# raw-lab/mercat2

Hardware: AMD Instinct MI355X
Metric: bases/sec at k=31, 10Mx150bp (higher is better)
Workload: dtype u64

## Files before the change

### mercat2_amd/csrc/mk_skmer.hip

```cpp
#include "mk_skmer_dev.h"
#include <cstdlib>
#include <cstdio>
#include <vector>
#include <type_traits>

#define SK_NKMAX 8
#ifndef SK_HIST_THREADS
#define SK_HIST_THREADS 256
#endif
#ifndef SK_HIST_GRID
#define SK_HIST_GRID 512
#endif
#ifndef SK_SCAT_GRID
#define SK_SCAT_GRID 4096
#endif
#define SK_MAX_P1_LOG2 13
#define SK_MAX_P1 (1 << SK_MAX_P1_LOG2)
#ifndef SK_BUCKET_SYMS
#define SK_BUCKET_SYMS 8192
#endif
#define SK_NOFIT 0xFF000000u

template <int W, class F>
__device__ __forceinline__ void sk_for_each_record(u64 w0, u64 w1, u64 badw, int k, int nkmax, bool canon, F&& emit) {
  const SkRuns r = sk_analyse<W>(w0, w1, sk_valid32(badw, k), canon);
  sk_walk(r, w0, w1, nkmax, canon, emit);
}

__device__ __forceinline__ ulonglong2 sk_make_record(u64 w0, u64 w1, int jstart, int nk, int k) {
  const int s = 2 * jstart;
  u64 hi = (w0 << s) | ((w1 >> 1) >> (63 - s));
  u64 lo = w1 << s;
  const int t = 2 * (nk + k - 1);
  const u64 mh = t >= 64 ? ~0ull : (~0ull << ((64 - t) & 63));
  const u64 ml = t <= 64 ? 0ull : (~0ull << ((128 - t) & 63));
  hi &= mh;
  lo = (lo & ml) | (u64)nk;
  return make_ulonglong2(hi, lo);
}

template <int W, bool CANON>
__global__ __launch_bounds__(SK_HIST_THREADS) void mk_sk_hist_k(const u64* __restrict__ codes, const u64* __restrict__ bad,
                                                                const MkChunkInfo* __restrict__ info, u64* __restrict__ hist,
                                                                u64* __restrict__ khist, int p1_log2, int k, int nkmax,
                                                                size_t nthreads_total, int canon, int sample_log2) {
  extern __shared__ unsigned sk_hist_lds[];
  (void)canon;
  sk_hist_body(sk_hist_lds, sk_hist_lds + (1u << p1_log2), info, hist, p1_log2, nthreads_total, sample_log2,
               [&](size_t t, size_t p0, auto&& tally) {
                 sk_for_each_record<W>(codes[t], codes[t + 1], bad_window(bad, p0), k, nkmax, CANON, tally);
               });
}

#ifndef SK_TU_CANON
__device__ __forceinline__ u64 sk_cap(u64 h, int sample_log2, u64 weight, float sigmas) {
  if (sample_log2 == 0) return h;
  const u64 est = h << sample_log2;
  const float dev = sigmas * __builtin_sqrtf((float)((u64)weight << sample_log2) * (float)est);
  return est + (u64)dev + 1 + (sigmas > 0 ? 16 * weight : 0);
}
__device__ __forceinline__ u64 sk_seg_cap(u64 h, int sample_log2, u64 weight, float sigmas, int nseg) {
  const float est = (float)(h << sample_log2);
  const float var = (float)weight * est * (1.0f / (float)nseg + (float)(1u << sample_log2) / (float)(nseg * nseg));
  return (u64)(est / (float)nseg) + (u64)(sigmas * __builtin_sqrtf(var)) + 1 + (sigmas > 0 ? 4 * weight : 0);
}
__global__ __launch_bounds__(1024) void mk_sk_scan_k(const u64* __restrict__ hist, const u64* __restrict__ khist,
                                                     u64* __restrict__ start, SkCursor* __restrict__ cursor, u64* __restrict__ kstart,
                                                     MkChunkInfo* __restrict__ info, int p1_log2, int sample_log2, int nkmax,
                                                     u64 div, u64 part_cap, u64 surv_cap, float sigmas, int nseg) {
  constexpr int PER = SK_MAX_P1 / 1024;
  __shared__ u64 wsum[16], wksum[16];
  const unsigned p1 = 1u << p1_log2;
  const unsigned per = (p1 + 1023) / 1024;
  const unsigned lo = threadIdx.x * per;
  const int lane = threadIdx.x & 63, wv = threadIdx.x >> 6;
  u64 cap[PER], kcap[PER];
  u64 acc = 0, kacc = 0;
#pragma unroll
  for (int q = 0; q < PER; ++q) {
    const unsigned i = lo + q;
    const bool on = (unsigned)q < per && i < p1;
    const u64 hk = on ? hist[i] : 0ull;
    cap[q] = !on ? 0 : (nseg > 1 ? sk_seg_cap(hk & 0xFFFFFFFFull, sample_log2, SK_R / SK_NKMAX, sigmas, 8)
                                 : sk_cap(hk & 0xFFFFFFFFull, sample_log2, SK_R / SK_NKMAX, sigmas));
    kcap[q] = on ? (sk_cap(hk >> 32, sample_log2, SK_R, sigmas) + div - 1) / div : 0;
    acc += cap[q];
    kacc += kcap[q];
  }
  u64 inc = acc, kinc = kacc;
#pragma unroll
  for (int d = 1; d < 64; d <<= 1) {
    const u64 a = __shfl_up(inc, d), b = __shfl_up(kinc, d);
    if (lane >= d) { inc += a; kinc += b; }
  }
  if (lane == 63) { wsum[wv] = inc; wksum[wv] = kinc; }
  __syncthreads();
  u64 run = inc - acc, krun = kinc - kacc;
  for (int w = 0; w < wv; ++w) { run += wsum[w]; krun += wksum[w]; }
  __shared__ u64 s_total;
  if (threadIdx.x == 1023) {
    const u64 total = run + acc, ktotal = krun + kacc;
    s_total = total;
    const u64 all = nseg > 1 ? 16 * total : total;
    start[(size_t)nseg * p1] = all;
    kstart[p1] = ktotal;
    if (all > part_cap) atomicOr(&info->part_overflow, 1ull);
    if (ktotal > surv_cap) atomicOr(&info->part_overflow, 2ull);
  }
  __shared__ unsigned s_run[SK_MAX_P1];
#pragma unroll
  for (int q = 0; q < PER; ++q) {
    const unsigned i = lo + q;
    if ((unsigned)q < per && i < p1) {
      s_run[i] = (unsigned)run;
      kstart[i] = krun;
      run += cap[q];
      krun += kcap[q];
    }
  }
  __syncthreads();
  const u64 total = s_total;
  for (int x = 0; x < nseg; ++x)
    for (unsigned i = threadIdx.x; i < p1; i += 1024) {
      const u64 at = x < 8 ? (u64)x * total + s_run[i] : 8 * total + 8 * (u64)s_run[i];
      start[(size_t)x * p1 + i] = at;
      cursor[(size_t)x * p1 + i] = (SkCursor)at;
    }
}

#endif

#ifdef MK_STAMP
static __device__ u64 skq_dbg[1024 * 8];
#endif
#define SKQ_CAP 512
#if defined(SK_ABL_COARSE) && !defined(SK_PLAIN_CURSORS)
#error "SK_ABL_COARSE needs -DSK_PLAIN_CURSORS (the ablation's region ends differ from the ones sk_reserve8k checks)"
#endif
#ifndef SKQ_THREADS
#define SKQ_THREADS 512
#endif
#define SKQ_WAVES (SKQ_THREADS / 64)
#define SKQ_WALKED 0xFFFFFFFFu
template <int W, bool CANON, int SKQ_SUBT, int SKQ_QCAP>
__global__ __launch_bounds__(SKQ_THREADS) __attribute__((amdgpu_waves_per_eu(4, 4))) void mk_sk_scatterq_k(const u64* __restrict__ codes, const u64* __restrict__ bad,
                                                         MkChunkInfo* __restrict__ info, const u64* __restrict__ start,
                                                         SkCursor* __restrict__ cursor, ulonglong2* __restrict__ part,
                                                         int p1_log2, int k, int nkmax, size_t ntiles, unsigned qcap, int nseg) {
  SkCursor* const shared_cursor = cursor + ((size_t)8 << p1_log2);
  const u64* const shared_start = start + ((size_t)8 << p1_log2);
  if (nseg > 1) {
    unsigned xcc;
    asm volatile("s_getreg_b32 %0, hwreg(HW_REG_XCC_ID)" : "=s"(xcc));
    const size_t seg = xcc & 7u;
    cursor += seg << p1_log2;
    start += seg << p1_log2;
  }
  __shared__ unsigned lh[SK_MAX_P1];
  __shared__ u64 pk_x[SKQ_SUBT][SKQ_WAVES][65];
  __shared__ unsigned queue[SKQ_SUBT][SKQ_WAVES][SKQ_QCAP];
  __shared__ unsigned s_abort;
  if (threadIdx.x == 0) s_abort = info->part_overflow != 0;
  __syncthreads();
  if (s_abort) return;
  unsigned spilled = 0;
  constexpr int NB = SK_MAX_P1 / SKQ_THREADS;
  const unsigned p1 = 1u << p1_log2;
  const size_t seq_len = info->seq_len;
  const int lane = threadIdx.x & 63;
#define wv sk_wave_id()
  auto sk_wave_id = [&]() { int w = (int)threadIdx.x; asm volatile("" : "+v"(w)); return w >> 6; };
  for (unsigned i = threadIdx.x; i < p1; i += blockDim.x) lh[i] = 0;
  __syncthreads();
  u64 tA = 0, tB = 0, tC = 0, tD = 0, tE = 0, tF = 0, t0 = 0, ntile = 0;
  (void)tA; (void)tB; (void)tC; (void)tD; (void)tE; (void)tF; (void)t0; (void)ntile;
  STAMP(t0);
  for (size_t tile = blockIdx.x; tile < ntiles; tile += gridDim.x) {
    ntile += 1;
    unsigned qn[SKQ_SUBT];
#pragma unroll
    for (int st = 0; st < SKQ_SUBT; ++st) {
      const size_t t = (tile * SKQ_SUBT + st) * SKQ_THREADS + threadIdx.x;
      const size_t p0 = t * SK_R;
      SkRuns runs;
      runs.valid = 0;
      runs.starts = 0;
      runs.pos[0] = runs.pos[1] = runs.pos[2] = runs.pos[3] = 0;
      u64 ww0 = 0, ww1 = 0;
      if (p0 < seq_len) {
        ww0 = codes[t];
        ww1 = codes[t + 1];
        runs = sk_analyse<W>(ww0, ww1, sk_valid32(bad_window(bad, p0), k), CANON);
      } else if (p0 < seq_len + SK_R) {
        ww0 = codes[t];
      }
      pk_x[st][wv][lane] = ww0;
      if (lane == 63) pk_x[st][wv][64] = ww1;
      const unsigned s2 = sk_cut_starts(runs.starts, runs.valid, nkmax);
      const unsigned cnt = __popc(s2);
      const unsigned inc = mk_wave_scan_incl(cnt);
      const unsigned total = mk_wave_last(inc);
      unsigned* const myq = queue[st][wv];
      if (total <= qcap) {
        unsigned todo = s2, at = inc - cnt;
        while (todo) {
          const int j = __ffs(todo) - 1;
          todo &= todo - 1;
          const unsigned stop = (s2 | ~runs.valid) & ~((2u << j) - 1);
          const int nk = (stop ? (__ffs(stop) - 1) : SK_R) - j;
          const u64 pw = j < 10 ? runs.pos[0] : (j < 20 ? runs.pos[1] : (j < 30 ? runs.pos[2] : runs.pos[3]));
          const unsigned best = (unsigned)(pw >> (6 * (j % 10))) & 63u;
          myq[at++] = (unsigned)lane | ((unsigned)j << 6) | ((unsigned)nk << 11) | (best << 16);
        }
        __builtin_amdgcn_fence(__ATOMIC_RELEASE, "wavefront");
        __builtin_amdgcn_wave_barrier();
        __builtin_amdgcn_fence(__ATOMIC_ACQUIRE, "wavefront");
        for (unsigned base = 0; base < total; base += 64) {
          const unsigned i = base + lane;
          if (i < total) {
            const unsigned it = myq[i];
            const u64* const wp = &pk_x[st][wv][it & 63u];
            const unsigned mm = sk_canon_mmer(sk_mmer(wp[0], wp[1], (int)(it >> 16)), CANON);
#ifdef SK_ABL_COARSE
            const unsigned b = sk_bucket(mm, p1_log2) & ~63u;
#else
            const unsigned b = sk_bucket(mm, p1_log2);
#endif
            atomicAdd(&lh[b], 1u);
            myq[i] = (it & 0xFFFFu) | (b << 16);
          }
        }
        qn[st] = total;
      } else {
        if (p0 < seq_len)
          sk_walk(runs, ww0, ww1, nkmax, CANON, [&](int, int, unsigned mm) {
            atomicAdd(&lh[sk_bucket(mm, p1_log2)], 1u);
          });
        qn[st] = SKQ_WALKED;
      }
    }
    STAMP_ADD(tA, t0);
    __syncthreads();
    STAMP_ADD(tB, t0);
    unsigned roff = 0;
    asm volatile("" : "+s"(roff));
    SkCursor* const rcursor = cursor + roff;
    const u64* const rstart = start + roff;
    SkCursor* const rshared_cursor = shared_cursor + roff;
    const u64* const rshared_start = shared_start + roff;
#ifndef SK_PLAIN_CURSORS
    if (p1 == SK_MAX_P1) {
      static_assert(NB % 8 == 0, "sk_reserve8");
#pragma unroll
      for (int h = 0; h < NB; h += 8) {
        unsigned v[8], at[8];
#pragma unroll
        for (int i = 0; i < 8; ++i) v[i] = lh[threadIdx.x + (h + i) * SKQ_THREADS];
        unsigned nofit = sk_reserve8<SKQ_THREADS>(v, rcursor + h * SKQ_THREADS, rstart + h * SKQ_THREADS, SK_NOFIT, at);
        if (nseg > 1 && __any(nofit)) {
          unsigned v2[8], at2[8];
#pragma unroll
          for (int i = 0; i < 8; ++i) {
            v2[i] = at[i] >= SK_NOFIT ? v[i] : 0u;
            const unsigned pad = at[i] >= SK_NOFIT ? at[i] & 0xFFFFFFu : 0u;
            if (pad) {
              const u64 end = rstart[threadIdx.x + (h + i) * SKQ_THREADS + 1];
              for (unsigned q = 0; q < pad; ++q) part[end - pad + q] = make_ulonglong2(0, 0);
            }
          }
          nofit = sk_reserve8<SKQ_THREADS>(v2, rshared_cursor + h * SKQ_THREADS, rshared_start + h * SKQ_THREADS, SK_NOFIT, at2);
#pragma unroll
          for (int i = 0; i < 8; ++i) at[i] = v2[i] ? at2[i] : at[i];
        }
        spilled |= nofit;
#pragma unroll
        for (int i = 0; i < 8; ++i) lh[threadIdx.x + (h + i) * SKQ_THREADS] = at[i];
      }
    } else
#endif
    {
      for (unsigned b = threadIdx.x; b < p1; b += SKQ_THREADS) {
        const unsigned v = lh[b];
        u64 r = v ? (u64)atomicAdd(&rcursor[b], v) : 0ull;
#ifdef SK_ABL_COARSE
        const bool fits = v == 0 || r + v <= rstart[b + 64 < p1 ? b + 64 : p1];
#else
        bool fits = v == 0 || r + v <= rstart[b + 1];
        if (!fits && nseg > 1) {
          for (u64 q = r; q < rstart[b + 1]; ++q) part[q] = make_ulonglong2(0, 0);
          r = (u64)atomicAdd(&rshared_cursor[b], v);
          fits = r + v <= rshared_start[b + 1];
        }
#endif
        spilled |= fits ? 0u : 1u;
        lh[b] = fits ? (unsigned)r : SK_NOFIT;
      }
    }
    STAMP_ADD(tC, t0);
    __syncthreads();
    STAMP_ADD(tD, t0);
#pragma unroll
    for (int st = 0; st < SKQ_SUBT; ++st) {
      if (qn[st] != SKQ_WALKED) {
        const unsigned total = qn[st];
        const unsigned* const myq = queue[st][wv];
        for (unsigned base = 0; base < total; base += 64) {
          const unsigned i = base + lane;
          if (i < total) {
            const unsigned it = myq[i];
            const unsigned at = atomicAdd(&lh[it >> 16], 1u);
            const u64* const wp = &pk_x[st][wv][it & 63u];
            ulonglong2 rec = sk_make_record(wp[0], wp[1], (int)((it >> 6) & 31u), (int)((it >> 11) & 31u), k);
            asm volatile("" : "+v"(rec.x), "+v"(rec.y));
            if (at < SK_NOFIT) part[(size_t)at] = rec;
          }
        }
      } else {
        const size_t t = (tile * SKQ_SUBT + st) * SKQ_THREADS + threadIdx.x;
        const size_t p0 = t * SK_R;
        if (p0 < seq_len) {
          const ulonglong2 w = make_ulonglong2(pk_x[st][wv][lane], pk_x[st][wv][lane + 1]);
          const SkRuns runs = sk_analyse<W>(w.x, w.y, sk_valid32(bad_window(bad, p0), k), CANON);
          sk_walk(runs, w.x, w.y, nkmax, CANON, [&](int jstart, int nk, unsigned mm) {
            const unsigned at = atomicAdd(&lh[sk_bucket(mm, p1_log2)], 1u);
            if (at < SK_NOFIT) part[(size_t)at] = sk_make_record(w.x, w.y, jstart, nk, k);
          });
        }
      }
    }
    STAMP_ADD(tE, t0);
    __syncthreads();
    for (unsigned i = threadIdx.x; i < p1; i += blockDim.x) lh[i] = 0;
    __syncthreads();
    STAMP_ADD(tF, t0);
  }
#ifdef MK_STAMP
  if (threadIdx.x == 0 && blockIdx.x < 1024) { u64* d = skq_dbg + (size_t)blockIdx.x * 8; d[0] = tA; d[1] = tB; d[2] = tC; d[3] = tD; d[4] = tE; d[5] = tF; d[6] = ntile; }
#endif
  if (spilled) atomicOr(&info->part_overflow, 4ull);
}
#undef wv


#ifndef SK_TU_CANON
void mk_launch_sk_scan(mk_ctx* c, const u64* hist, const u64* khist, u64* start, SkCursor* cursor, u64* kstart, int p1_log2,
                       int sample_log2, int nkmax, u64 surv_div, u64 part_cap, u64 surv_cap, float sigmas, int nseg) {
  hipLaunchKernelGGL(mk_sk_scan_k, dim3(1), dim3(1024), 0, c->stream, hist, khist, start, cursor, kstart,
                     (MkChunkInfo*)c->info.p, p1_log2, sample_log2, nkmax, surv_div, part_cap, surv_cap, sigmas, nseg);
}

#endif

template <int W, bool CANON>
static void launch_wc(mk_ctx* c, size_t seq_len, int p1_log2, int nkmax, int sample_log2, u64 surv_div, u64 part_cap, u64 surv_cap,
                     u64* hist, u64* start, SkCursor* cursor, u64* khist, u64* kstart, bool reuse, int nseg) {
  MkChunkInfo* info = (MkChunkInfo*)c->info.p;
  const size_t threads = div_up(seq_len, SK_R);
  const size_t tiles = div_up(div_up(threads, (size_t)1 << sample_log2), SK_HIST_THREADS);
  const size_t hist_grid = sample_log2 ? SK_HIST_GRID / 2 : SK_HIST_GRID;
  if (!reuse) {
    const float sigmas = (float)mk_env_double("MK_SAMPLE_SIGMAS", 6.0);
    hipLaunchKernelGGL((mk_sk_hist_k<W, CANON>), dim3((unsigned)(tiles < hist_grid ? tiles : hist_grid)), dim3(SK_HIST_THREADS),
                       2 * sizeof(unsigned) << p1_log2, c->stream,
                       (const u64*)c->codes.p, (const u64*)c->bad.p, info, hist, khist, p1_log2, c->k, nkmax, threads, c->canonical,
                       sample_log2);
    mk_launch_sk_scan(c, (const u64*)hist, (const u64*)khist, start, cursor, kstart, p1_log2, sample_log2, nkmax, surv_div, part_cap,
                      surv_cap, sigmas, nseg);
  }
  const SkQueueShape shape = sk_queue_shape(c);
  const bool three = shape.three;
  const unsigned qcap = shape.qcap;
  const size_t qtiles = div_up(threads, (size_t)SKQ_THREADS * (three ? 3 : 2));
  const dim3 qgrid((unsigned)(qtiles < SK_SCAT_GRID ? qtiles : SK_SCAT_GRID));
  if (three)
    hipLaunchKernelGGL((mk_sk_scatterq_k<W, CANON, 3, 376>), qgrid, dim3(SKQ_THREADS), 0, c->stream, (const u64*)c->codes.p,
                       (const u64*)c->bad.p, info, (const u64*)start, cursor, (ulonglong2*)c->part.p, p1_log2, c->k, nkmax, qtiles, qcap, nseg);
  else
    hipLaunchKernelGGL((mk_sk_scatterq_k<W, CANON, 2, 512>), qgrid, dim3(SKQ_THREADS), 0, c->stream, (const u64*)c->codes.p,
                       (const u64*)c->bad.p, info, (const u64*)start, cursor, (ulonglong2*)c->part.p, p1_log2, c->k, nkmax, qtiles, qcap, nseg);
#ifdef MK_STAMP
  {
    (void)hipStreamSynchronize(c->stream);
    const unsigned g = qgrid.x;
    std::vector<u64> h(8 * 1024);
    (void)hipMemcpyFromSymbol(h.data(), HIP_SYMBOL(skq_dbg), h.size() * 8);
    double a[7] = {0, 0, 0, 0, 0, 0, 0};
    for (unsigned w = 0; w < g && w < 1024; ++w) for (int q = 0; q < 7; ++q) a[q] += (double)h[w * 8 + q] / g;
    fprintf(stderr, "[stamp scatterq] per WG (wave 0): analyse+list+pass1=%.0f barrier1=%.0f cursors=%.0f barrier2=%.0f pass2=%.0f barrier3+clear=%.0f tiles=%.2f grid=%u\n",
            a[0], a[1], a[2], a[3], a[4], a[5], a[6], g);
  }
#endif
}


template <bool CANON>
static bool sk_partition(int W, mk_ctx* c, size_t seq_len, int p1_log2, int nkmax, int sample_log2, u64 surv_div, u64 part_cap, u64 surv_cap,
                         u64* hist, u64* start, SkCursor* cursor, u64* khist, u64* kstart, bool reuse, int nseg) {
  switch (W) {
#define SK_CASE(W_)                                                                                                      \
  case W_: launch_wc<W_, CANON>(c, seq_len, p1_log2, nkmax, sample_log2, surv_div, part_cap, surv_cap, hist, start, cursor, khist, kstart, reuse, nseg); return true;
    SK_CASE(2) SK_CASE(3) SK_CASE(4) SK_CASE(5) SK_CASE(6) SK_CASE(7)
    SK_CASE(8) SK_CASE(9) SK_CASE(10) SK_CASE(11) SK_CASE(12) SK_CASE(13) SK_CASE(14) SK_CASE(15) SK_CASE(16)
    SK_CASE(17) SK_CASE(18) SK_CASE(19) SK_CASE(20) SK_CASE(21) SK_CASE(22)
#undef SK_CASE
    default: return false;
  }
}

#ifdef SK_TU_CANON
bool mk_sk_partition_canon(int W, mk_ctx* c, size_t seq_len, int p1_log2, int nkmax, int sample_log2, u64 surv_div, u64 part_cap,
                           u64 surv_cap, u64* hist, u64* start, SkCursor* cursor, u64* khist, u64* kstart, bool reuse, int nseg) {
  return sk_partition<true>(W, c, seq_len, p1_log2, nkmax, sample_log2, surv_div, part_cap, surv_cap, hist, start, cursor, khist, kstart, reuse, nseg);
}
#else
bool mk_sk_partition_canon(int W, mk_ctx* c, size_t seq_len, int p1_log2, int nkmax, int sample_log2, u64 surv_div, u64 part_cap,
                           u64 surv_cap, u64* hist, u64* start, SkCursor* cursor, u64* khist, u64* kstart, bool reuse, int nseg);

bool mk_part_inherit(mk_ctx* c, size_t seq_len, int p1_log2, uint64_t min_count, bool sampled, bool exact) {
  if (c->part_cooldown > 0 && !exact) c->part_cooldown -= 1;
  const bool reuse = !exact && sampled && c->part_reuse_ok && !c->part_dirty && c->part_cooldown == 0 &&
                     p1_log2 == c->part_prev_p1 && (unsigned long long)min_count == c->part_prev_minc &&
                     seq_len <= c->part_prev_len + c->part_prev_len / 100 && seq_len >= c->part_prev_len - c->part_prev_len / 50 &&
                     !mk_env_set("MK_NO_REUSE");
  if (reuse) c->st.part_reused += 1;
  c->part_dirty = true;
  if (exact) { c->part_reuse_ok = false; c->part_cooldown = 4; }
  else if (sampled && !reuse) {
    c->part_reuse_ok = true;
    c->part_prev_len = seq_len;
    c->part_prev_p1 = p1_log2;
    c->part_prev_minc = (unsigned long long)min_count;
  } else if (!reuse) c->part_reuse_ok = false;
  return reuse;
}

int sk_p1_log2(size_t seq_len, int max_log2, size_t bucket_syms) {
  int p1_log2 = 8;
  while (p1_log2 < max_log2 && (seq_len >> p1_log2) > bucket_syms) ++p1_log2;
  return p1_log2;
}
int sk_sample_log2(size_t seq_len, bool exact) {
  return !exact && seq_len >= (size_t)mk_env_int("MK_SAMPLE_MIN", (long long)8 << 20) ? 3 : 0;
}
u64 sk_surv_div(uint64_t min_count) { return min_count > 1 ? (u64)min_count : 1; }
size_t sk_surv_cap(size_t seq_len, size_t p1, u64 surv_div, int sample_log2) {
  if (!sample_log2) return seq_len / surv_div + p1 + 64;
  const double L = 1.25 * (double)seq_len, S = (double)(1u << sample_log2), w = (double)SK_R;
  return (size_t)((L + 6.0 * sqrt((double)p1 * S * w * L) + 16.0 * w * (double)p1) / (double)surv_div) + 2 * p1 + 64;
}
SkQueueShape sk_queue_shape(const mk_ctx* c) {
  const long long force_subt = mk_env_int("MK_SKQ_SUBT", 0);
  SkQueueShape q;
  q.three = force_subt == 3 || (force_subt != 2 && c->items_hint > 0 && c->items_hint * 64.0 + 48.0 < 376.0);
  q.qcap = q.three ? 376u : 512u;
  { const long long v = mk_env_int("MK_SKQ_CAP", -1); if (v >= 0 && (unsigned long long)v < q.qcap) q.qcap = (unsigned)v; }
  return q;
}

int mk_launch_count_superkmer(mk_ctx* c, size_t seq_len, uint64_t min_count, bool exact) {
  if (seq_len == 0) return MK_OK;
  const int k = c->k;
  const int p1_log2 = sk_p1_log2(seq_len, SK_MAX_P1_LOG2, SK_BUCKET_SYMS);
  c->p1_log2 = p1_log2;
  const size_t p1 = (size_t)1 << p1_log2;
  int nkmax = 62 - k;
  if (nkmax > SK_NKMAX) nkmax = SK_NKMAX;
  { const long long v = mk_env_int("MK_NKMAX", 0); if (v >= 1 && v <= 31 && v <= 62 - k) nkmax = (int)v; }
  const int sample_log2 = sk_sample_log2(seq_len, exact);
  c->part_sampled = sample_log2 != 0;
  const int nseg = (sample_log2 != 0 && seq_len <= ((size_t)1 << 30) && mk_env_int("MK_XSEG", 1) != 0) ? 9 : 1;
  if (nseg != c->part_nseg) c->part_reuse_ok = false;
  c->part_nseg = nseg;
  const bool reuse = mk_part_inherit(c, seq_len, p1_log2, min_count, sample_log2 != 0, exact);
  int rc;
  if ((rc = mk_buf_reserve(c, c->part_meta, sk_meta_words(p1, SKC_SEG_MAX) * sizeof(u64))) != MK_OK) return rc;
  const size_t part_cap = nseg > 1 ? 2 * seq_len + 64 : seq_len + 64;
  if ((rc = mk_buf_reserve(c, c->part, part_cap * sizeof(ulonglong2))) != MK_OK) return rc;
  const u64 surv_div = sk_surv_div(min_count);
  const size_t surv_cap = sk_surv_cap(seq_len, p1, surv_div, sample_log2);
  if ((rc = mk_buf_reserve(c, c->surv_keys, surv_cap * sizeof(u64))) != MK_OK) return rc;
  if ((rc = mk_buf_reserve(c, c->surv_cnts, surv_cap * sizeof(u64))) != MK_OK) return rc;
  const SkMeta m = sk_meta(c->part_meta.p, p1, nseg);
  if (!reuse) MK_HIP(hipMemsetAsync(m.hist, 0, sk_meta_cleared_words(p1) * sizeof(u64), c->stream));
  mk_prof_begin(c, MK_K_PART);
  if (c->canonical) {
    if (!mk_sk_partition_canon(k - SK_M + 1, c, seq_len, p1_log2, nkmax, sample_log2, surv_div, (u64)part_cap, (u64)surv_cap, m.hist, m.start, m.cursor, m.khist, m.kstart, reuse, nseg)) {
      c->err = "mk_launch_count_superkmer: k out of range";
      return MK_ERR_ARG;
    }
  } else if (!sk_partition<false>(k - SK_M + 1, c, seq_len, p1_log2, nkmax, sample_log2, surv_div, (u64)part_cap, (u64)surv_cap, m.hist, m.start, m.cursor, m.khist, m.kstart, reuse, nseg)) {
    c->err = "mk_launch_count_superkmer: k out of range";
    return MK_ERR_ARG;
  }
  mk_prof_end(c);
  if ((rc = mk_launch_sk_count(c, (const u64*)m.start, m.cursor, (const u64*)m.kstart, m.nsurv, min_count, p1, nseg)) != MK_OK) return rc;
  MK_HIP(hipGetLastError());
  c->surv_regions = 1;
  return MK_OK;
}
#endif
```

### mercat2_amd/csrc/mk_skmer_dev.h

```cpp
#pragma once
#include "mk_common.h"
#include "mk_device.h"

#define SK_M 11
#define SK_MASK ((1u << (2 * SK_M)) - 1)
#define SK_R 32

__device__ __forceinline__ unsigned sk_order_raw(unsigned mm) {
  return __umul24(mm, 0x9277B5u) + 0x2C5A3Du;
}
__device__ __forceinline__ unsigned sk_order_hash(unsigned mm) { return sk_order_raw(mm) & SK_MASK; }
__device__ __forceinline__ unsigned sk_canon_mmer(unsigned mm, bool canon) {
  if (!canon) return mm;
  const unsigned rc = (unsigned)mk_revcomp2((u64)mm, SK_M);
  return rc < mm ? rc : mm;
}
__device__ __forceinline__ unsigned sk_bucket(unsigned mm, int p1_log2) { return (mm * 0xC2B2AE3Du) >> (32 - p1_log2); }

__device__ __forceinline__ unsigned sk_mmer(u64 w0, u64 w1, int q) {
  const u64 a = q < 32 ? w0 : w1, b = q < 32 ? w1 : 0ull;
  const int s = 2 * (q & 31);
  const u64 x = (a << s) | ((b >> 1) >> (63 - s));
  return (unsigned)(x >> (64 - 2 * SK_M));
}

typedef unsigned SkCursor;

#ifndef SK_PLAIN_CURSORS
template <int THREADS>
__device__ __forceinline__ unsigned sk_reserve8(const unsigned (&count)[8], SkCursor* cursor, const u64* start, unsigned nofit,
                                                unsigned (&base)[8]) {
  unsigned r[8];
  u64 lim[8];
  const unsigned voff4 = threadIdx.x * 4u, voff8 = threadIdx.x * 8u;
#pragma unroll
  for (int i = 0; i < 8; ++i) {
    u64 saved;
    r[i] = 0;
    asm volatile(
        "v_cmp_ne_u32 vcc, 0, %3\n\t"
        "s_and_saveexec_b64 %1, vcc\n\t"
        "s_nop 4\n\t"
        "global_atomic_add %0, %2, %3, %4 sc0\n\t"
        "s_mov_b64 exec, %1"
        : "+v"(r[i]), "=&s"(saved)
        : "v"(voff4), "v"(count[i]), "s"(cursor + i * THREADS)
        : "memory", "vcc", "scc");
  }
#pragma unroll
  for (int i = 0; i < 8; ++i)
    asm volatile("s_nop 4\n\tglobal_load_dwordx2 %0, %1, %2 offset:8" : "=&v"(lim[i]) : "v"(voff8), "s"(start + i * THREADS) : "memory");
  asm volatile("s_waitcnt vmcnt(0)"
               : "+v"(r[0]), "+v"(r[1]), "+v"(r[2]), "+v"(r[3]), "+v"(r[4]), "+v"(r[5]), "+v"(r[6]), "+v"(r[7]), "+v"(lim[0]),
                 "+v"(lim[1]), "+v"(lim[2]), "+v"(lim[3]), "+v"(lim[4]), "+v"(lim[5]), "+v"(lim[6]), "+v"(lim[7])
               :
               : "memory");
  unsigned spilled = 0;
#pragma unroll
  for (int i = 0; i < 8; ++i) {
    const bool fits = count[i] == 0 || (u64)r[i] + count[i] <= lim[i];
    spilled |= fits ? 0u : 1u;
    base[i] = fits ? r[i] : nofit | ((u64)r[i] < lim[i] ? (unsigned)(lim[i] - r[i]) : 0u);
  }
  return spilled;
}
#endif

template <int THREADS, int MAX_P1>
__device__ __forceinline__ void sk_reserve_tile(unsigned* count, unsigned* base, SkCursor* cursor, const u64* start, unsigned p1,
                                                unsigned nofit, unsigned& spilled) {
#ifndef SK_PLAIN_CURSORS
  if (p1 == MAX_P1) {
    constexpr int NB = MAX_P1 / THREADS;
    static_assert(NB % 8 == 0, "sk_reserve8");
#pragma unroll
    for (int h = 0; h < NB; h += 8) {
      unsigned v[8], at[8];
#pragma unroll
      for (int i = 0; i < 8; ++i) v[i] = count[threadIdx.x + (h + i) * THREADS];
      spilled |= sk_reserve8<THREADS>(v, cursor + h * THREADS, start + h * THREADS, nofit, at);
#pragma unroll
      for (int i = 0; i < 8; ++i) {
        base[threadIdx.x + (h + i) * THREADS] = at[i];
        if (base != count) count[threadIdx.x + (h + i) * THREADS] = 0;
      }
    }
  } else
#endif
  {
    for (unsigned b = threadIdx.x; b < p1; b += THREADS) {
      const unsigned v = count[b];
      const u64 r = v ? (u64)atomicAdd(&cursor[b], v) : 0ull;
      const bool fits = v == 0 || r + v <= start[b + 1];
      spilled |= fits ? 0u : 1u;
      base[b] = fits ? (unsigned)r : nofit;
      if (base != count) count[b] = 0;
    }
  }
}

__device__ __forceinline__ unsigned sk_valid32(u64 badw, int k) {
  if (badw == 0) return ~0u;
  u64 d = badw;
  int cover = 1;
  while (2 * cover <= k) { d |= d >> cover; cover *= 2; }
  if (cover < k) d |= d >> (k - cover);
  return ~(unsigned)d;
}

struct SkRuns {
  unsigned valid, starts;
  u64 pos[4];
};

template <int W>
__device__ __forceinline__ SkRuns sk_analyse(u64 w0, u64 w1, unsigned valid, bool canon) {
  constexpr int NQ = SK_R + W - 1;
  unsigned ord[NQ];
  {
    unsigned mm = sk_mmer(w0, w1, 0);
#pragma unroll
    for (int q = 0; q < NQ; ++q) {
      if (q) {
        const int pos = q + SK_M - 1;
        const unsigned base = (unsigned)((pos < 32 ? (w0 >> (62 - 2 * pos)) : (w1 >> (62 - 2 * (pos - 32)))) & 3u);
        mm = ((mm << 2) | base) & SK_MASK;
      }
      unsigned h = sk_order_raw(sk_canon_mmer(mm, canon));
      asm("" : "+v"(h));
      ord[q] = (h << 10) | (unsigned)q;
    }
  }
  constexpr int WA = W >= 3 ? 3 : 1, WB = W >= 9 ? 9 : WA;
  if constexpr (W >= 3) {
#pragma unroll
    for (int q = 0; q + 2 < NQ; ++q) ord[q] = min(min(ord[q], ord[q + 1]), ord[q + 2]);
  }
  if constexpr (W >= 9) {
#pragma unroll
    for (int q = 0; q + 8 < NQ; ++q) ord[q] = min(min(ord[q], ord[q + 3]), ord[q + 6]);
  }
  static_assert(W <= 3 * WB, "a third round of minima would be needed");
  SkRuns r;
  r.valid = valid;
  r.starts = 0;
  r.pos[0] = r.pos[1] = r.pos[2] = r.pos[3] = 0;
  unsigned prev_pos = 64;
#pragma unroll
  for (int j = 0; j < SK_R; ++j) {
    const bool ok = (valid >> j) & 1u;
    unsigned best;
    if constexpr (W == WB) best = ord[j];
    else if constexpr (W <= 2 * WB) best = min(ord[j], ord[j + W - WB]);
    else best = min(min(ord[j], ord[j + WB]), ord[j + W - WB]);
    best &= 63u;
    r.starts |= (ok && best != prev_pos) ? (1u << j) : 0u;
    prev_pos = ok ? best : 64u;
    r.pos[j / 10] |= (u64)best << (6 * (j % 10));
  }
  return r;
}

template <class F>
__device__ __forceinline__ void sk_walk(const SkRuns& r, u64 w0, u64 w1, int nkmax, bool canon, F&& emit) {
  unsigned todo = r.starts;
  while (todo) {
    const int j = __ffs(todo) - 1;
    todo &= todo - 1;
    const unsigned stop = (r.starts | ~r.valid) & ~((2u << j) - 1);
    int nk = (stop ? (__ffs(stop) - 1) : SK_R) - j;
    const u64 pw = j < 10 ? r.pos[0] : (j < 20 ? r.pos[1] : (j < 30 ? r.pos[2] : r.pos[3]));
    const unsigned best = (unsigned)(pw >> (6 * (j % 10))) & 63u;
    const unsigned mm = sk_canon_mmer(sk_mmer(w0, w1, (int)best), canon);
    int at = j;
    while (nk > 0) {
      const int take = nk < nkmax ? nk : nkmax;
      emit(at, take, mm);
      at += take;
      nk -= take;
    }
  }
}

__device__ __forceinline__ unsigned sk_cut_starts(unsigned starts, unsigned valid, int nkmax) {
  if (nkmax >= SK_R) return starts;
  const unsigned cont = valid & ~starts;
  unsigned a = cont;
  int len = 1;
  while (2 * len <= nkmax) { a &= a << len; len *= 2; }
  if (len < nkmax) a &= a << (nkmax - len);
  unsigned s2 = starts;
  for (unsigned c = (starts << nkmax) & a; c; c = (c << nkmax) & a) s2 |= c;
  return s2;
}

template <class A>
__device__ __forceinline__ void sk_hist_body(unsigned* lh, unsigned* lk, const MkChunkInfo* __restrict__ info, u64* __restrict__ hist,
                                             int p1_log2, size_t nthreads_total, int sample_log2, A&& analyse) {
  const unsigned p1 = 1u << p1_log2, nthr = blockDim.x;
  for (unsigned i = threadIdx.x; i < p1; i += nthr) { lh[i] = 0; lk[i] = 0; }
  __syncthreads();
  const size_t seq_len = info->seq_len;
  const size_t ngroups = (nthreads_total + ((size_t)1 << sample_log2) - 1) >> sample_log2;
  for (size_t g = (size_t)blockIdx.x * nthr + threadIdx.x; g < ngroups; g += (size_t)gridDim.x * nthr) {
    size_t t = g;
    if (sample_log2) t = (g << sample_log2) + (((unsigned)g * 0x9E3779B1u >> 7) & ((1u << sample_log2) - 1));
    const size_t p0 = t * SK_R;
    if (t >= nthreads_total || p0 >= seq_len) continue;
    analyse(t, p0, [&](int, int nk, unsigned mm) {
      const unsigned b = sk_bucket(mm, p1_log2);
      atomicAdd(&lh[b], 1u);
      atomicAdd(&lk[b], (unsigned)nk);
    });
  }
  __syncthreads();
  for (unsigned b = threadIdx.x; b < p1; b += nthr) {
    const unsigned v = lh[b];
    if (v) atomicAdd(&hist[b], (u64)v | ((u64)lk[b] << 32));
  }
}

#define SKC_SEG_WORDS 20
#define SKC_SEG_MAX 9
__device__ __forceinline__ unsigned skc_seg_at(const unsigned* tab, unsigned j, int nseg) {
  if (nseg == 1) return tab[10] + j;
  const uint4 a = *reinterpret_cast<const uint4*>(tab), b = *reinterpret_cast<const uint4*>(tab + 4);
  const unsigned c = tab[8];
  unsigned x = 0;
#define SKC_SEG_STEP(P) asm("v_cmp_le_u32 vcc, %1, %2\n\tv_addc_co_u32 %0, vcc, 0, %0, vcc" : "+v"(x) : "v"(P), "v"(j) : "vcc")
  SKC_SEG_STEP(a.y); SKC_SEG_STEP(a.z); SKC_SEG_STEP(a.w); SKC_SEG_STEP(b.x); SKC_SEG_STEP(b.y); SKC_SEG_STEP(b.z); SKC_SEG_STEP(b.w);
  SKC_SEG_STEP(c);
#undef SKC_SEG_STEP
  return tab[10 + x] + j;
}
__device__ __forceinline__ void skc_seg_publish(unsigned* tab, unsigned seg_lo, unsigned seg_hi, unsigned seg_end, int nseg) {
  asm volatile("" : "+v"(seg_lo), "+v"(seg_hi), "+v"(seg_end));
  const unsigned x = threadIdx.x & 15u, cnt = x < (unsigned)nseg ? (seg_hi < seg_end ? seg_hi : seg_end) - seg_lo : 0u;
  unsigned inc = cnt;
  inc += (unsigned)__builtin_amdgcn_update_dpp(0, (int)inc, 0x111, 0xf, 0xf, false);
  inc += (unsigned)__builtin_amdgcn_update_dpp(0, (int)inc, 0x112, 0xf, 0xf, false);
  inc += (unsigned)__builtin_amdgcn_update_dpp(0, (int)inc, 0x114, 0xf, 0xf, false);
  inc += (unsigned)__builtin_amdgcn_update_dpp(0, (int)inc, 0x118, 0xf, 0xf, false);
  if (x < SKC_SEG_MAX) {
    tab[x] = inc - cnt;
    tab[10 + x] = seg_lo - (inc - cnt);
  }
  if (x == 15) tab[9] = inc;
}

#ifdef MK_STAMP
#define STAMP(var) { __builtin_amdgcn_sched_barrier(0); unsigned long long t__; asm volatile("s_memtime %0\n\ts_waitcnt lgkmcnt(0)" : "=s"(t__) :: "memory"); __builtin_amdgcn_sched_barrier(0); var = t__; }
#define STAMP_ADD(acc, t0) { unsigned long long t1__; STAMP(t1__); acc += t1__ - t0; t0 = t1__; }
#else
#define STAMP(var)
#define STAMP_ADD(acc, t0)
#endif
```

Measured before the change: 166.7 billion.

## Merge super-k-mers spanning adjacent thread windows via DPP lane exchange

Adds a cross-lane span step to the scatter kernel. Each lane receives its left neighbour's trailing-run state through DPP. When the minimizer position matches, the lane drops its own leading start, and the neighbour extends its last super-k-mer into this window, reading a third word when building the record. The aim is fewer, longer super-k-mer records, which means fewer atomics and less partition traffic in later stages. In exchange it adds per-tile DPP work, a reciprocal-based phase computation, and more complicated record boundaries that could break correctness at wave edges.

```diff
diff --git a/mercat2_amd/csrc/mk_skmer.hip b/mercat2_amd/csrc/mk_skmer.hip
--- a/mercat2_amd/csrc/mk_skmer.hip
+++ b/mercat2_amd/csrc/mk_skmer.hip
@@ -27,16 +27,19 @@
   sk_walk(r, w0, w1, nkmax, canon, emit);
 }
 
-__device__ __forceinline__ ulonglong2 sk_make_record(u64 w0, u64 w1, int jstart, int nk, int k) {
+__device__ __forceinline__ ulonglong2 sk_make_record(u64 w0, u64 w1, u64 w2, int jstart, int nk, int k) {
   const int s = 2 * jstart;
   u64 hi = (w0 << s) | ((w1 >> 1) >> (63 - s));
-  u64 lo = w1 << s;
+  u64 lo = (w1 << s) | ((w2 >> 1) >> (63 - s));
   const int t = 2 * (nk + k - 1);
   const u64 mh = t >= 64 ? ~0ull : (~0ull << ((64 - t) & 63));
   const u64 ml = t <= 64 ? 0ull : (~0ull << ((128 - t) & 63));
   hi &= mh;
   lo = (lo & ml) | (u64)nk;
   return make_ulonglong2(hi, lo);
+}
+__device__ __forceinline__ ulonglong2 sk_make_record(u64 w0, u64 w1, int jstart, int nk, int k) {
+  return sk_make_record(w0, w1, 0ull, jstart, nk, k);
 }
 
 template <int W, bool CANON>
@@ -146,7 +149,7 @@
 __global__ __launch_bounds__(SKQ_THREADS) __attribute__((amdgpu_waves_per_eu(4, 4))) void mk_sk_scatterq_k(const u64* __restrict__ codes, const u64* __restrict__ bad,
                                                          MkChunkInfo* __restrict__ info, const u64* __restrict__ start,
                                                          SkCursor* __restrict__ cursor, ulonglong2* __restrict__ part,
-                                                         int p1_log2, int k, int nkmax, size_t ntiles, unsigned qcap, int nseg) {
+                                                         int p1_log2, int k, int nkmax, size_t ntiles, unsigned qcap, int nseg, int span) {
   SkCursor* const shared_cursor = cursor + ((size_t)8 << p1_log2);
   const u64* const shared_start = start + ((size_t)8 << p1_log2);
   if (nseg > 1) {
@@ -168,6 +171,7 @@
   const unsigned p1 = 1u << p1_log2;
   const size_t seq_len = info->seq_len;
   const int lane = threadIdx.x & 63;
+  const unsigned nk_recip = 65535u / (unsigned)nkmax + 1u;
 #define wv sk_wave_id()
   auto sk_wave_id = [&]() { int w = (int)threadIdx.x; asm volatile("" : "+v"(w)); return w >> 6; };
   for (unsigned i = threadIdx.x; i < p1; i += blockDim.x) lh[i] = 0;
@@ -196,7 +200,16 @@
       }
       pk_x[st][wv][lane] = ww0;
       if (lane == 63) pk_x[st][wv][64] = ww1;
-      const unsigned s2 = sk_cut_starts(runs.starts, runs.valid, nkmax);
+      unsigned st2 = runs.starts, seed = 0, ext = 0;
+      if (span)
+        seed = sk_span_in((unsigned)__builtin_amdgcn_update_dpp(0, (int)sk_span_out(runs), 0x138, 0xf, 0xf, false), st2, runs.valid,
+                          (unsigned)runs.pos[0] & 63u, nkmax, nk_recip);
+      const unsigned s2 = sk_cut_starts(st2, runs.valid, nkmax, seed);
+      if (span) {
+        const unsigned ends = s2 | ~runs.valid;
+        const unsigned mine = (runs.starts & ~st2 & 1u) ? (unsigned)__ffs((int)ends) - 1u : 0u;
+        ext = (unsigned)__builtin_amdgcn_update_dpp(0, (int)mine, 0x130, 0xf, 0xf, false);
+      }
       const unsigned cnt = __popc(s2);
       const unsigned inc = mk_wave_scan_incl(cnt);
       const unsigned total = mk_wave_last(inc);
@@ -207,7 +220,7 @@
           const int j = __ffs(todo) - 1;
           todo &= todo - 1;
           const unsigned stop = (s2 | ~runs.valid) & ~((2u << j) - 1);
-          const int nk = (stop ? (__ffs(stop) - 1) : SK_R) - j;
+          const int nk = (stop ? (__ffs(stop) - 1) : SK_R + (int)ext) - j;
           const u64 pw = j < 10 ? runs.pos[0] : (j < 20 ? runs.pos[1] : (j < 30 ? runs.pos[2] : runs.pos[3]));
           const unsigned best = (unsigned)(pw >> (6 * (j % 10))) & 63u;
           myq[at++] = (unsigned)lane | ((unsigned)j << 6) | ((unsigned)nk << 11) | (best << 16);
@@ -310,7 +323,8 @@
             const unsigned it = myq[i];
             const unsigned at = atomicAdd(&lh[it >> 16], 1u);
             const u64* const wp = &pk_x[st][wv][it & 63u];
-            ulonglong2 rec = sk_make_record(wp[0], wp[1], (int)((it >> 6) & 31u), (int)((it >> 11) & 31u), k);
+            const u64 w2 = pk_x[st][wv][(it & 63u) < 62u ? (it & 63u) + 2u : 64u];
+            ulonglong2 rec = sk_make_record(wp[0], wp[1], w2, (int)((it >> 6) & 31u), (int)((it >> 11) & 31u), k);
             asm volatile("" : "+v"(rec.x), "+v"(rec.y));
             if (at < SK_NOFIT) part[(size_t)at] = rec;
           }
@@ -353,7 +367,7 @@
 
 template <int W, bool CANON>
 static void launch_wc(mk_ctx* c, size_t seq_len, int p1_log2, int nkmax, int sample_log2, u64 surv_div, u64 part_cap, u64 surv_cap,
-                     u64* hist, u64* start, SkCursor* cursor, u64* khist, u64* kstart, bool reuse, int nseg) {
+                     u64* hist, u64* start, SkCursor* cursor, u64* khist, u64* kstart, bool reuse, int nseg, int span) {
   MkChunkInfo* info = (MkChunkInfo*)c->info.p;
   const size_t threads = div_up(seq_len, SK_R);
   const size_t tiles = div_up(div_up(threads, (size_t)1 << sample_log2), SK_HIST_THREADS);
@@ -374,10 +388,10 @@
   const dim3 qgrid((unsigned)(qtiles < SK_SCAT_GRID ? qtiles : SK_SCAT_GRID));
   if (three)
     hipLaunchKernelGGL((mk_sk_scatterq_k<W, CANON, 3, 376>), qgrid, dim3(SKQ_THREADS), 0, c->stream, (const u64*)c->codes.p,
-                       (const u64*)c->bad.p, info, (const u64*)start, cursor, (ulonglong2*)c->part.p, p1_log2, c->k, nkmax, qtiles, qcap, nseg);
+                       (const u64*)c->bad.p, info, (const u64*)start, cursor, (ulonglong2*)c->part.p, p1_log2, c->k, nkmax, qtiles, qcap, nseg, span);
   else
     hipLaunchKernelGGL((mk_sk_scatterq_k<W, CANON, 2, 512>), qgrid, dim3(SKQ_THREADS), 0, c->stream, (const u64*)c->codes.p,
-                       (const u64*)c->bad.p, info, (const u64*)start, cursor, (ulonglong2*)c->part.p, p1_log2, c->k, nkmax, qtiles, qcap, nseg);
+                       (const u64*)c->bad.p, info, (const u64*)start, cursor, (ulonglong2*)c->part.p, p1_log2, c->k, nkmax, qtiles, qcap, nseg, span);
 #ifdef MK_STAMP
   {
     (void)hipStreamSynchronize(c->stream);
@@ -395,10 +409,10 @@
 
 template <bool CANON>
 static bool sk_partition(int W, mk_ctx* c, size_t seq_len, int p1_log2, int nkmax, int sample_log2, u64 surv_div, u64 part_cap, u64 surv_cap,
-                         u64* hist, u64* start, SkCursor* cursor, u64* khist, u64* kstart, bool reuse, int nseg) {
+                         u64* hist, u64* start, SkCursor* cursor, u64* khist, u64* kstart, bool reuse, int nseg, int span) {
   switch (W) {
 #define SK_CASE(W_)                                                                                                      \
-  case W_: launch_wc<W_, CANON>(c, seq_len, p1_log2, nkmax, sample_log2, surv_div, part_cap, surv_cap, hist, start, cursor, khist, kstart, reuse, nseg); return true;
+  case W_: launch_wc<W_, CANON>(c, seq_len, p1_log2, nkmax, sample_log2, surv_div, part_cap, surv_cap, hist, start, cursor, khist, kstart, reuse, nseg, span); return true;
     SK_CASE(2) SK_CASE(3) SK_CASE(4) SK_CASE(5) SK_CASE(6) SK_CASE(7)
     SK_CASE(8) SK_CASE(9) SK_CASE(10) SK_CASE(11) SK_CASE(12) SK_CASE(13) SK_CASE(14) SK_CASE(15) SK_CASE(16)
     SK_CASE(17) SK_CASE(18) SK_CASE(19) SK_CASE(20) SK_CASE(21) SK_CASE(22)
@@ -409,12 +423,12 @@
 
 #ifdef SK_TU_CANON
 bool mk_sk_partition_canon(int W, mk_ctx* c, size_t seq_len, int p1_log2, int nkmax, int sample_log2, u64 surv_div, u64 part_cap,
-                           u64 surv_cap, u64* hist, u64* start, SkCursor* cursor, u64* khist, u64* kstart, bool reuse, int nseg) {
-  return sk_partition<true>(W, c, seq_len, p1_log2, nkmax, sample_log2, surv_div, part_cap, surv_cap, hist, start, cursor, khist, kstart, reuse, nseg);
+                           u64 surv_cap, u64* hist, u64* start, SkCursor* cursor, u64* khist, u64* kstart, bool reuse, int nseg, int span) {
+  return sk_partition<true>(W, c, seq_len, p1_log2, nkmax, sample_log2, surv_div, part_cap, surv_cap, hist, start, cursor, khist, kstart, reuse, nseg, span);
 }
 #else
 bool mk_sk_partition_canon(int W, mk_ctx* c, size_t seq_len, int p1_log2, int nkmax, int sample_log2, u64 surv_div, u64 part_cap,
-                           u64 surv_cap, u64* hist, u64* start, SkCursor* cursor, u64* khist, u64* kstart, bool reuse, int nseg);
+                           u64 surv_cap, u64* hist, u64* start, SkCursor* cursor, u64* khist, u64* kstart, bool reuse, int nseg, int span);
 
 bool mk_part_inherit(mk_ctx* c, size_t seq_len, int p1_log2, uint64_t min_count, bool sampled, bool exact) {
   if (c->part_cooldown > 0 && !exact) c->part_cooldown -= 1;
@@ -472,6 +486,7 @@
   if (nseg != c->part_nseg) c->part_reuse_ok = false;
   c->part_nseg = nseg;
   const bool reuse = mk_part_inherit(c, seq_len, p1_log2, min_count, sample_log2 != 0, exact);
+  const int span = mk_env_int("MK_SK_SPAN", 1) != 0 ? 1 : 0;
   int rc;
   if ((rc = mk_buf_reserve(c, c->part_meta, sk_meta_words(p1, SKC_SEG_MAX) * sizeof(u64))) != MK_OK) return rc;
   const size_t part_cap = nseg > 1 ? 2 * seq_len + 64 : seq_len + 64;
@@ -484,11 +499,11 @@
   if (!reuse) MK_HIP(hipMemsetAsync(m.hist, 0, sk_meta_cleared_words(p1) * sizeof(u64), c->stream));
   mk_prof_begin(c, MK_K_PART);
   if (c->canonical) {
-    if (!mk_sk_partition_canon(k - SK_M + 1, c, seq_len, p1_log2, nkmax, sample_log2, surv_div, (u64)part_cap, (u64)surv_cap, m.hist, m.start, m.cursor, m.khist, m.kstart, reuse, nseg)) {
+    if (!mk_sk_partition_canon(k - SK_M + 1, c, seq_len, p1_log2, nkmax, sample_log2, surv_div, (u64)part_cap, (u64)surv_cap, m.hist, m.start, m.cursor, m.khist, m.kstart, reuse, nseg, span)) {
       c->err = "mk_launch_count_superkmer: k out of range";
       return MK_ERR_ARG;
     }
-  } else if (!sk_partition<false>(k - SK_M + 1, c, seq_len, p1_log2, nkmax, sample_log2, surv_div, (u64)part_cap, (u64)surv_cap, m.hist, m.start, m.cursor, m.khist, m.kstart, reuse, nseg)) {
+  } else if (!sk_partition<false>(k - SK_M + 1, c, seq_len, p1_log2, nkmax, sample_log2, surv_div, (u64)part_cap, (u64)surv_cap, m.hist, m.start, m.cursor, m.khist, m.kstart, reuse, nseg, span)) {
     c->err = "mk_launch_count_superkmer: k out of range";
     return MK_ERR_ARG;
   }
diff --git a/mercat2_amd/csrc/mk_skmer_dev.h b/mercat2_amd/csrc/mk_skmer_dev.h
--- a/mercat2_amd/csrc/mk_skmer_dev.h
+++ b/mercat2_amd/csrc/mk_skmer_dev.h
@@ -182,16 +182,31 @@
   }
 }
 
-__device__ __forceinline__ unsigned sk_cut_starts(unsigned starts, unsigned valid, int nkmax) {
-  if (nkmax >= SK_R) return starts;
+__device__ __forceinline__ unsigned sk_cut_starts(unsigned starts, unsigned valid, int nkmax, unsigned seed = 0) {
+  if (nkmax >= SK_R) return starts | seed;
   const unsigned cont = valid & ~starts;
   unsigned a = cont;
   int len = 1;
   while (2 * len <= nkmax) { a &= a << len; len *= 2; }
   if (len < nkmax) a &= a << (nkmax - len);
-  unsigned s2 = starts;
-  for (unsigned c = (starts << nkmax) & a; c; c = (c << nkmax) & a) s2 |= c;
+  unsigned s2 = starts | seed;
+  for (unsigned c = (s2 << nkmax) & a; c; c = (c << nkmax) & a) s2 |= c;
   return s2;
+}
+
+__device__ __forceinline__ unsigned sk_span_out(const SkRuns& r) {
+  const unsigned pos31 = (unsigned)(r.pos[3] >> 6) & 63u;
+  return (r.valid >> 31) | (pos31 << 1) | (((unsigned)__clz((int)r.starts) + 1u) << 7);
+}
+__device__ __forceinline__ unsigned sk_span_in(unsigned in, unsigned& starts, unsigned valid, unsigned pos0, int nkmax,
+                                               unsigned nk_recip) {
+  const unsigned ends = (starts & ~1u) | ~valid;
+  const bool go = (in & 1u) && (valid & 1u) && ends != 0 && pos0 + SK_R == ((in >> 1) & 63u);
+  if (!go) return 0u;
+  starts &= ~1u;
+  const unsigned c = in >> 7, phase = c - ((c * nk_recip) >> 16) * (unsigned)nkmax;
+  const unsigned j0 = phase ? (unsigned)nkmax - phase : 0u, e = (unsigned)__ffs((int)ends) - 1u;
+  return j0 < e ? 1u << j0 : 0u;
 }
 
 template <class A>
```

New measurement: 171.2 billion, median of 6. 1.03x the previous value.
